# CarbonMatrixLab/AbX

Measured on AMD Instinct MI355X. Metric: diffusion-steps/sec (100 samples, ~350-res complex), higher is better.
Workload: dtype f32; 1 GPU; L352: L=352 (Lab 228 + antigen 124), 100 samples of one complex over 1 GPU(s), 1 step = ScoreNetwork (3 passes) + get_prev + reverse, seeded random weights, ESM off; L=352, samples_total=100, chunk=auto, parallelism=sample-shard x1, no collective in the step

## Files before the change

### abx_amd/csrc/gemm3.hip

```cpp
#include "common.h"
#include "abx_hip.h"
#include "gemm_epilogue.h"
#include "rigid_dev.h"

namespace {

constexpr int BK = 16;
#ifndef ABX_SPLIT_MIN_TILES
#define ABX_SPLIT_MIN_TILES 256
#endif
typedef __attribute__((address_space(3))) void* lds_ptr_t;
typedef const __attribute__((address_space(1))) void* glb_ptr_t;

__device__ __forceinline__ void glds16(const void* src, char* dst_wave_base) {
    __builtin_amdgcn_global_load_lds((glb_ptr_t)src, (lds_ptr_t)dst_wave_base, 16, 0, 0);
}

__device__ __forceinline__ unsigned vgpr32(unsigned o) {
    asm volatile("" : "+v"(o));
    return o;
}

template <int N> __device__ __forceinline__ void wait_vm_and_barrier() {
    asm volatile("s_waitcnt vmcnt(%0) lgkmcnt(0)\n\ts_barrier" ::"n"(N) : "memory");
}

template <int ROWS>
__device__ __forceinline__ int plane_off(int plane, int row, int half) {
    return plane * (ROWS * 32) + row * 32 + ((half ^ ((row >> 3) & 1)) << 4);
}

template <int ROWS, int NL, int NPL = 2>
__device__ __forceinline__ void plane_sources(long long s_plane, long long s_row, int r0, int R, unsigned (&off)[NL]) {
    const int lane = threadIdx.x & 63, wave = threadIdx.x >> 6;
#pragma unroll
    for (int i = 0; i < NL; ++i) {
        int o = (wave * NL + i) * 1024 + lane * 16;
        if (o >= NPL * ROWS * 32) o -= NPL * ROWS * 32;
        const int plane = o / (ROWS * 32), rem = o % (ROWS * 32);
        const int row = rem >> 5, hp = (rem >> 4) & 1;
        const int half = hp ^ ((row >> 3) & 1);
        const int gr = min(r0 + row, R - 1);
        off[i] = (unsigned)((plane * s_plane + (long long)gr * s_row + 8 * half) * 2);
    }
}

template <int BM, int BN, int WM, int WN, int AMODE, bool SWAP = false, bool STATS = true, int RING = 2, int JGO = 0>
__device__ __forceinline__ void gemm3_mainloop(const AbxGemm& g, float* smem, int mt, int nt, int b, f32x16 (&acc)[WM / 32][WN / 32],
                                               float (&ls)[WM / 32], float (&lq)[WM / 32], float (&lshift)[WM / 32],
                                               const char* a_lds = nullptr, int a_lds_stride = 0) {
    constexpr int TM = WM / 32, TN = WN / 32;
    constexpr int WAVES_N = BN / WN;
    constexpr int A_IMG = AMODE == 3 ? 0 : (AMODE == 2 ? 2 * BM * 32 : BM * 64);
    constexpr int NLA = AMODE == 3 ? 1 : (A_IMG + 4095) / 4096;
    constexpr int A_STAGE = RING == 2 ? A_IMG : (A_IMG + 4095) / 4096 * 4096;
    constexpr int B_IMG = 2 * BN * 32;
// ... 528 lines not shown
#pragma unroll
                    for (int q = 0; q < 2; ++q) {
                        const int hc = hid0 + j * 32 + 8 * (2 * s2 + q) + 4 * h;
                        const int hcl = min(hc, MLP_NH - 4);
                        const f32x4 cs = *reinterpret_cast<const f32x4*>(cst + hcl), bi = *reinterpret_cast<const f32x4*>(cst + MLP_NH + hcl);
#pragma unroll
                        for (int e = 0; e < 4; ++e) {
                            float x = rstd * (acc1[0][j][8 * s2 + 4 * q + e] - dmean * cs[e]) + bi[e];
                            x = relu_keep_nan(x);
                            v[4 * q + e] = (hc + e < g.N) ? x : 0.f;
                        }
                    }
                    unsigned q0[4], q1[4];
#pragma unroll
                    for (int e = 0; e < 4; ++e) split2b(v[2 * e], v[2 * e + 1], q0[e], q1[e]);
                    hf[0] = u32x4{q0[0], q0[1], q0[2], q0[3]};
                    hf[1] = u32x4{q1[0], q1[1], q1[2], q1[3]};
                }
                const int kl = 2 * j + s2;
                const int knext = c * (BN / 16) + kl + 1;
                if (kl + 1 < BN / 16 && knext * 16 < g.N) issue_w2(knext, (kl + 1) & 1);
                const char* ws = W2s + (kl & 1) * B2_IMG + offB2;
                if (rows_live && (c * (BN / 16) + kl) * 16 < g.N) {
#pragma unroll
                    for (int t0 = 0; t0 < TN2; t0 += TG2) {
                        u32x4 wb[TG2][2];
#pragma unroll
                        for (int t = 0; t < TG2; ++t)
#pragma unroll
                            for (int p = 0; p < 2; ++p) wb[t][p] = *reinterpret_cast<const u32x4*>(ws + (t0 + t) * 1024 + p * (BN2 * 32));
                        constexpr int TA[3] = {1, 0, 0}, TB[3] = {0, 1, 0};
#pragma unroll
                        for (int term = 0; term < 3; ++term)
#pragma unroll
                            for (int t = 0; t < TG2; ++t)
                                acc2[0][t0 + t] = mfma_split(hf[TA[term]], wb[t][TB[term]], acc2[0][t0 + t]);
                    }
                }
                wait_vm_and_barrier<0>();
            }
        }
    }
    {
        const float cs2 = __builtin_ldexpf(1.0f, -4 - g.b2_exp);
#pragma unroll
        for (int t = 0; t < TN2; ++t) acc2[0][t] *= cs2;
    }
    AbxGemm g2 = g;
    g2.N = g.N2; g2.bias = g.bias2; g2.ln_csum = nullptr; g2.ln_stats = nullptr; g2.act = 0; g2.alpha = 1.0f;
    __syncthreads();
    gemm_epilogue<BM, BN2, WM, BN2, EDGE, false>(g2, smem, smem + 2 * BM, acc2, mt * BM, 0, b, false);
}

template <int MINB>
__global__ __launch_bounds__(256, MINB) void gemm3_mlp_kernel(const AbxGemm g) {
    constexpr int OPER = (2 * 128 * 64 + 2 * 2 * 128 * 32 + 2 * 2 * 192 * 32) / 4 + 2 * MLP_NH;
    constexpr int EPI = 2 * 128 + 4 * 32 * (3 * 32 + 4);
    __shared__ __attribute__((aligned(16))) float smem[OPER > EPI ? OPER : EPI];
    const int ntm = (g.M + 127) / 128;
    const unsigned nwg = gridDim.x, bid = blockIdx.x;
    const unsigned q = nwg >> 3, r = nwg & 7, xcd = bid & 7, loc = bid >> 3;
    const unsigned wgid = (xcd < r ? xcd * (q + 1) : r * (q + 1) + (xcd - r) * q) + loc;
    const int b = (int)(wgid / (unsigned)ntm), mt = (int)(wgid - (unsigned)b * (unsigned)ntm);
    const ClockProbe probe(g.clock_probe);
    if ((mt + 1) * 128 <= g.M && g.N2 == 192) gemm3_mlp_block<false>(g, smem, mt, b);
    else gemm3_mlp_block<true>(g, smem, mt, b);
    probe.finish();
}

constexpr int MLP3_LDS = 3 * (128 * 64 + 2 * 128 * 32) + 2 * 2 * 192 * 32 + 2 * MLP_NH * 4;
__global__ __launch_bounds__(256, 2) void gemm3_mlp3_kernel(const AbxGemm g) {
    extern __shared__ __attribute__((aligned(16))) float mlp3_smem[];
    const int ntm = (g.M + 127) / 128;
    const unsigned nwg = gridDim.x, bid = blockIdx.x;
    const unsigned q = nwg >> 3, r = nwg & 7, xcd = bid & 7, loc = bid >> 3;
    const unsigned wgid = (xcd < r ? xcd * (q + 1) : r * (q + 1) + (xcd - r) * q) + loc;
    const int b = (int)(wgid / (unsigned)ntm), mt = (int)(wgid - (unsigned)b * (unsigned)ntm);
    const ClockProbe probe(g.clock_probe);
    if ((mt + 1) * 128 <= g.M && g.N2 == 192) gemm3_mlp_block<false, 3>(g, mlp3_smem, mt, b);
    else gemm3_mlp_block<true, 3>(g, mlp3_smem, mt, b);
    probe.finish();
}

constexpr int GT_NG = 192;
template <bool EDGE>
__device__ __forceinline__ void gemm3_gtail2w_block(const AbxGemm& g, float* smem, int mt, int b) {
    constexpr int BM = 128, BN = 96, WM = 32, WN = 96, BN2 = 192, TN2 = BN2 / 32;
    constexpr int G1_BYTES = 2 * BM * 64 + 2 * 2 * BN * 32;
    constexpr int B2_IMG = 2 * BN2 * 32;
    constexpr int NL2 = (B2_IMG + 4095) / 4096;
    constexpr int G_IMG = BM * 64;
    char* W2s = reinterpret_cast<char*>(smem) + G1_BYTES;
    char* Gs = W2s + 2 * B2_IMG;
    float* cst = reinterpret_cast<float*>(Gs + 3 * G_IMG);
    for (int i = threadIdx.x; i < GT_NG; i += 256) {
        cst[i] = i < g.N ? g.ln_csum[i] : 0.f;
        cst[GT_NG + i] = (i < g.N && g.bias) ? g.bias[i] : 0.f;
    }
    const int lane = threadIdx.x & 63, wave = __builtin_amdgcn_readfirstlane(threadIdx.x >> 6), h = lane >> 5;
    const int m0 = mt * BM;
    f32x16 acc2[1][TN2];
#pragma unroll
    for (int t = 0; t < TN2; ++t)
#pragma unroll
        for (int r = 0; r < 16; ++r) acc2[0][t][r] = 0.f;
    unsigned offs2[NL2];
    plane_sources<BN2, NL2>(g.sB23p, g.sB23n, 0, g.N2, offs2);
    const char* base2 = reinterpret_cast<const char*>(g.B2_split);
    const long long step2 = g.sB23k * 2;
    unsigned offsG[2];
    const char* baseG = reinterpret_cast<const char*>(g.gate + (long long)b * g.sGb + (long long)m0 * g.sGm);
#pragma unroll
    for (int i = 0; i < 2; ++i) {
        const int r = (wave * 2 + i) * 16 + (lane >> 2), p = lane & 3;
        const int kq = p ^ ((r >> 2) & 3);
        const int gri = min(m0 + r, g.M - 1) - m0;
        offsG[i] = (unsigned)(((long long)gri * g.sGm + kq * 4) * 4);
    }
    static_assert(B2_IMG % 4096 == 0, "uniform DMA instruction counts per wave (counted waits)");
    auto issue_w2 = [&](int ktile) {
        char* dst = W2s + (ktile & 1) * B2_IMG + wave * NL2 * 1024;
        const char* src = base2 + ktile * step2;
#pragma unroll
        for (int i = 0; i < NL2; ++i) glds16(src + vgpr32(offs2[i]), dst + i * 1024);
    };
    const int nkt2 = g.N / 16;
    auto issue_g = [&](int ktile) {
        const int kt = min(ktile, nkt2 - 1);
        char* dg = Gs + (ktile % 3) * G_IMG + wave * 2048;
        const char* sg = baseG + kt * 64;
#pragma unroll
        for (int i = 0; i < 2; ++i) glds16(sg + vgpr32(offsG[i]), dg + i * 1024);
    };
    const int offB2 = plane_off<BN2>(0, lane & 31, h);
// ... 589 lines not shown
    }
    if (!g.A_split && g.sAk == 1 && ((g.a_pair_transpose > 0 || g.a_pair) ? (long long)g.M * g.sAm : 128LL * g.sAm) >= (1LL << 30)) return 1;
    if (g.pair_Lp > 0 && g.c_pair && g.c_transposed) return 1;
    if (g.a_pair && (g.A_split || g.sAk != 1)) return 1;
    if (!g.A_split && g.sAk != 1 && 16LL * g.sAk + g.M >= (1LL << 30)) return 1;
    if (((long long)g.M + 127) / 128 * (((long long)g.N + 127) / 128) * g.batch >= (1LL << 31)) return 1;
    if (g.A_split && (long long)(g.K / 16) * g.sA3k >= (1LL << 31)) return 1;
    if ((long long)(g.K / 16) * g.sB3k >= (1LL << 31)) return 1;
    if (g.out_ln_w) {
        if (g.N > 128 || g.c_transposed || g.C_split || g.A2 || g.A_split || g.sAk != 1 || !g.out_ln_b) {
            abx_set_error("abx_gemm: out_ln needs N <= 128, a k-contiguous fp32 A and a plain store (split-f16 path)");
            *rc = ABX_ERR_ARG;
            return 0;
        }
        const long long mt = ((long long)g.M + 127) / 128;
        hipLaunchKernelGGL((gemm3_oln_kernel<128, 128, 32, 128, 4>), dim3((unsigned)(mt * g.batch)), dim3(256), 0, st, g);
        *rc = abx_check_launch("abx_gemm(out_ln)");
        return 0;
    }
    if (g.mlp == 2) {
        if (g.A_split || g.sAk != 1 || g.c_transposed || g.C_split || g.glu || g.A2 || g.out_ln_w || !g.B2_split || g.N2 <= 0 || g.N2 > 192 ||
            g.N % 16 != 0 || g.N > GT_NG || g.act != 2 || g.alpha != 1.0f || g.rowscale || !g.gate || !g.ln_csum || g.ln_stats || g.a_relu ||
            g.a_pair_transpose > 0 || g.pair_Lp > 0 || !al16(g.B2_split) || g.sB23n % 8 != 0 || g.sB23p % 8 != 0 || g.sB23k % 8 != 0 ||
            (long long)(g.N / 16) * g.sB23k >= (1LL << 31) || !al16(g.ln_csum) || (g.bias && !al16(g.bias)) || !al16(g.gate) || g.sGm % 4 != 0 ||
            g.sGb % 4 != 0 || 128LL * g.sGm >= (1LL << 30)) {
            abx_set_error("abx_gemm: mlp = 2 (gated tail) needs a k-contiguous fp32 A with folded LayerNorm, act = 2, a 16-byte aligned gate "
                          "operand [M][N], N % 16 == 0, N2 <= 192, plain store, B2_split planes in the permuted k order");
            *rc = ABX_ERR_ARG;
            return 0;
        }
        const long long mt = ((long long)g.M + 127) / 128;
        if (g.tune & 64) {
            if (int e = abx_ensure_dynamic_lds(reinterpret_cast<const void*>(&gemm3_gtail2w_kernel), GT_LDS, "abx_gemm(gated tail)")) { *rc = e; return 0; }
            hipLaunchKernelGGL(gemm3_gtail2w_kernel, dim3((unsigned)(mt * g.batch)), dim3(256), GT_LDS, st, g);
            *rc = abx_check_launch("abx_gemm(gated tail, two walks)");
            return 0;
        }
        if (int e = abx_ensure_dynamic_lds(reinterpret_cast<const void*>(&gemm3_gtail_kernel), GT1_LDS, "abx_gemm(gated tail)")) { *rc = e; return 0; }
        hipLaunchKernelGGL(gemm3_gtail_kernel, dim3((unsigned)(mt * g.batch)), dim3(256), GT1_LDS, st, g);
        *rc = abx_check_launch("abx_gemm(gated tail)");
        return 0;
    }
    if (g.mlp) {
        if (g.A_split || g.sAk != 1 || g.c_transposed || g.C_split || g.glu || g.A2 || g.out_ln_w || !g.B2_split || g.N2 <= 0 || g.N2 > 192 ||
            g.N % 16 != 0 || g.N > MLP_NH || g.act != 1 || g.alpha != 1.0f || g.rowscale || g.gate || !g.ln_csum || g.ln_stats || g.a_relu ||
            g.a_pair_transpose > 0 || g.pair_Lp > 0 || !al16(g.B2_split) || g.sB23n % 8 != 0 || g.sB23p % 8 != 0 || g.sB23k % 8 != 0 ||
            (long long)(g.N / 16) * g.sB23k >= (1LL << 31) || !al16(g.ln_csum) || (g.bias && !al16(g.bias))) {
            abx_set_error("abx_gemm: mlp needs a k-contiguous fp32 A with folded LayerNorm, relu, N % 16 == 0, N <= 768, N2 <= 192, plain store, "
                          "B2_split planes in the permuted k order");
            *rc = ABX_ERR_ARG;
            return 0;
        }
        const long long mt = ((long long)g.M + 127) / 128;
        if ((g.tune >> 5) & 1) {
            if (int e = abx_ensure_dynamic_lds(reinterpret_cast<const void*>(&gemm3_mlp3_kernel), MLP3_LDS, "abx_gemm(mlp)")) { *rc = e; return 0; }
            hipLaunchKernelGGL(gemm3_mlp3_kernel, dim3((unsigned)(mt * g.batch)), dim3(256), MLP3_LDS, st, g);
        } else if ((g.tune >> 4) & 1) hipLaunchKernelGGL(gemm3_mlp_kernel<1>, dim3((unsigned)(mt * g.batch)), dim3(256), 0, st, g);
        else hipLaunchKernelGGL(gemm3_mlp_kernel<2>, dim3((unsigned)(mt * g.batch)), dim3(256), 0, st, g);
        *rc = abx_check_launch("abx_gemm(mlp)");
        return 0;
    }
    if (g.A2) {
        if (g.A_split || g.c_transposed || g.glu || !g.B2_split || g.K2 % 16 != 0 || !al16(g.A2) || g.sA2m % 4 != 0 || g.sA2b % 4 != 0 ||
            !al16(g.B2_split) || g.sB23n % 8 != 0 || g.sB23p % 8 != 0 || g.sB23k % 8 != 0 || !g.ln2_csum ||
            (g.pair_Lp > 0 ? (long long)g.pair_L * g.pair_L * g.sA2m : 128LL * g.sA2m) >= (1LL << 30) ||
            (long long)(g.K2 / 16) * g.sB23k >= (1LL << 31)) {
            abx_set_error("abx_gemm: dual (A2 / B2_split) operands do not qualify for the split-f16 dual kernel");
            *rc = ABX_ERR_ARG;
            return 0;
        }
        const long long mt = ((long long)g.M + 127) / 128, ntn = ((long long)g.N + 95) / 96;
        if (g.N > 96 && g.N <= 192 && (g.tune & 128)) hipLaunchKernelGGL(gemm3_dual1_kernel, dim3((unsigned)(mt * g.batch)), dim3(256), 0, st, g);
        else if (g.tune & 1024) hipLaunchKernelGGL((gemm3_dual_kernel<128, 96, 32, 96, 4>), dim3((unsigned)(mt * ntn * g.batch)), dim3(256), 0, st, g);
        else hipLaunchKernelGGL((gemm3_dual_kernel<128, 96, 32, 96, 3>), dim3((unsigned)(mt * ntn * g.batch)), dim3(256), 0, st, g);
        *rc = abx_check_launch("abx_gemm(dual)");
        return 0;
    }
    if (narrow) {
        const long long mt = ((long long)g.M + 127) / 128;
        dim3 grid((unsigned)(mt * g.batch), 1, 1), block(256);
        if ((g.tune >> 9) & 3) {
            const int v = (g.tune >> 9) & 3;
            if (g.c_transposed) { if (v == 1) hipLaunchKernelGGL((gemm3_narrow_ring_kernel<true, 3, 4>), grid, block, 0, st, g); else hipLaunchKernelGGL((gemm3_narrow_ring_kernel<true, 4, 3>), grid, block, 0, st, g); }
            else { if (v == 1) hipLaunchKernelGGL((gemm3_narrow_ring_kernel<false, 3, 4>), grid, block, 0, st, g); else hipLaunchKernelGGL((gemm3_narrow_ring_kernel<false, 4, 3>), grid, block, 0, st, g); }
            *rc = abx_check_launch("abx_gemm(narrow, ring)");
            return 0;
        }
        if (g.c_transposed) hipLaunchKernelGGL((gemm3_kernel<128, 32, 32, 32, 0, true, 6>), grid, block, 0, st, g);
        else hipLaunchKernelGGL((gemm3_kernel<128, 32, 32, 32, 0, false, 6>), grid, block, 0, st, g);
        *rc = abx_check_launch("abx_gemm(narrow)");
        return 0;
    }
    const long long pad128 = ((g.N + 127) / 128) * 128, pad192 = ((g.N + 191) / 192) * 192;
    const int force = (g.tune >> 1) & 7;
    const bool wide = g.glu ? false : force ? force == 2 : (g.A_split ? pad192 <= pad128 : (pad192 <= pad128 && g.N % 128 != 0));
    const long long ntn128 = ((long long)g.N + 127) / 128;
    if (!wide && !g.glu && !force && mt128 * ntn128 * g.batch < 384 && g.M > 64) *rc = launch3<64, 128, 32, 64, 4>(g, st);
    else if (wide) *rc = launch3<128, 192, 32, 192, 3>(g, st);
    else *rc = launch3<128, 128, 32, 128, 4>(g, st);
    return 0;
}

int abx_gemm3_side_dispatch(const AbxGemm& g, const AbxGemm& s2, hipStream_t st, int* rc) {
    auto al16 = [](const void* p) { return (reinterpret_cast<uintptr_t>(p) & 15) == 0; };
    auto plain_a = [&](const AbxGemm& d) {
        return d.B_split && d.b_f16 && !d.A_split && d.A && d.sAk == 1 && d.K % 16 == 0 && al16(d.A) && d.sAm % 4 == 0 && d.sAb % 4 == 0 &&
               al16(d.B_split) && d.sB3n % 8 == 0 && d.sB3p % 8 == 0 && d.sB3k % 8 == 0 && d.sB3b % 8 == 0 && d.b_exp >= -100 && d.b_exp <= 100 &&
               !d.glu && !d.C_split && !d.A2 && !d.out_ln_w && !d.mlp && d.a_pair_transpose <= 0 && d.pair_Lp == 0 && d.batch_inner == 0 &&
               128LL * d.sAm < (1LL << 30) && (long long)(d.K / 16) * d.sB3k < (1LL << 31) && d.exact != 1;
    };
    if (!plain_a(g) || !plain_a(s2)) return 1;
// ... 79 lines not shown
```

### abx_amd/csrc/gemm_as.hip

```cpp
#include <stdlib.h>

#include <type_traits>

#include "common.h"
#include "abx_hip.h"

namespace {

typedef __attribute__((address_space(3))) void* lds_ptr_t;
typedef const __attribute__((address_space(1))) void* glb_ptr_t;

constexpr int AS_BM = 64, AS_BN = 128, AS_NK = 12, AS_RING = 3;
constexpr int AS_KT = 4096;
constexpr int AS_A = AS_NK * AS_KT;
constexpr int AS_STAGE = 2 * AS_BN * 32;
constexpr int AS_HALF = AS_KT / 2;
constexpr int AS_OFF_RING = AS_A;
constexpr int AS_OFF_ST = AS_OFF_RING + AS_RING * AS_STAGE;
constexpr int AS_OFF_CONST = AS_OFF_ST + 4 * 64 * 4;
constexpr int AS_LDS = AS_OFF_CONST + 2 * 1024;

__device__ __forceinline__ void as_glds16(const void* src, char* dst_wave_base) {
    __builtin_amdgcn_global_load_lds((glb_ptr_t)src, (lds_ptr_t)dst_wave_base, 16, 0, 0);
}
__device__ __forceinline__ unsigned as_vgpr32(unsigned o) {
    asm volatile("" : "+v"(o));
    return o;
}
template <int I> using IC = std::integral_constant<int, I>;
template <int I0, int I1, class F> __device__ __forceinline__ void as_static_for(F&& f) {
    if constexpr (I0 < I1) {
        f(IC<I0>{});
        as_static_for<I0 + 1, I1>(f);
    }
}

template <int ROWS> __device__ __forceinline__ int as_plane_off(int plane, int row, int half) {
    return plane * (ROWS * 32) + row * 32 + ((half ^ ((row >> 3) & 1)) << 4);
}

__device__ __forceinline__ long long as_a_row(const AbxGemm& g, int gri) {
    long long gr = gri;
    if (g.a_pair) {
        int pi, pj;
        if (g.c_split_tile) {
            pair_tile_decode(gri, g.pair_Lp, pi, pj);
            pi = min(pi, g.pair_L - 1);
            pj = min(pj, g.pair_L - 1);
        } else {
            pi = gri / g.pair_Lp;
            pj = min(gri - pi * g.pair_Lp, g.pair_L - 1);
        }
        gr = g.a_pair_transpose > 0 ? (long long)pj * g.pair_L + pi : (long long)pi * g.pair_L + pj;
    } else if (g.a_pair_transpose > 0) {
        const int qi = gri / g.a_pair_transpose;
        gr = (long long)(gri - qi * g.a_pair_transpose) * g.a_pair_transpose + qi;
    }
    return gr;
}

__device__ __forceinline__ void as_issue_a(const AbxGemm& g, char* lds, int m0, int b, int wm) {
    const int lane = threadIdx.x & 63;
    const bool remap = g.a_pair_transpose > 0 || g.a_pair != 0;
    const long long row0 = remap ? 0 : m0;
    const char* baseA = reinterpret_cast<const char*>(g.A + (long long)b * g.sAb + row0 * g.sAm);
    unsigned offA[2];
#pragma unroll
    for (int i = 0; i < 2; ++i) {
        const int r = 16 * i + (lane >> 2), p = lane & 3;
        const int kq = p ^ ((r >> 2) & 3);
        const long long gr = as_a_row(g, min(m0 + wm * 32 + r, g.M - 1));
        offA[i] = (unsigned)(((gr - row0) * g.sAm + kq * 4) * 4);
    }
    char* dst = lds + wm * AS_HALF;
#pragma unroll
    for (int kt = 0; kt < AS_NK; ++kt)
#pragma unroll
        for (int i = 0; i < 2; ++i) as_glds16(baseA + kt * 64 + as_vgpr32(offA[i]), dst + kt * AS_KT + i * 1024);
}

struct AsConv {
    float lshift, m2048;
    f32x2 ls2, lq2;
    int rd0, rd1, wr;
    bool ln, relu;
};
__device__ __forceinline__ void as_conv_init(AsConv& c, const AbxGemm& g) {
    const int lane = threadIdx.x & 63, r = lane & 31, h = lane >> 5, x = (r >> 2) & 3;
    c.rd0 = r * 64 + (((2 * h) ^ x) << 4);
    c.rd1 = r * 64 + (((2 * h + 1) ^ x) << 4);
    c.wr = as_plane_off<32>(0, r, h);
    c.lshift = 0.f;
    c.ls2 = c.lq2 = (f32x2){0.f, 0.f};
    c.m2048 = -2048.0f;
    asm volatile("" : "+v"(c.m2048));
    c.ln = g.ln_csum != nullptr;
    c.relu = g.a_relu != 0;
}
template <bool FIRST>
__device__ __forceinline__ void as_conv_ktile(AsConv& c, char* img) {
    const int lane = threadIdx.x & 63;
    const f32x4 lo = *reinterpret_cast<const f32x4*>(img + c.rd0);
    const f32x4 hi = *reinterpret_cast<const f32x4*>(img + c.rd1);
    float xv[8];
#pragma unroll
    for (int e = 0; e < 4; ++e) { xv[e] = lo[e]; xv[4 + e] = hi[e]; }
    if (c.ln) {
        if (FIRST) c.lshift = __shfl(xv[0], lane & 31, 64);
        const f32x2 sh2 = {c.lshift, c.lshift};
#pragma unroll
        for (int e = 0; e < 4; ++e) {
            f32x2 xp = {xv[2 * e], xv[2 * e + 1]};
            xp -= sh2;
            c.ls2 += xp;
            c.lq2 = __builtin_elementwise_fma(xp, xp, c.lq2);
            xv[2 * e] = xp[0];
            xv[2 * e + 1] = xp[1];
        }
    }
    if (c.relu) {
#pragma unroll
        for (int e = 0; e < 8; ++e) xv[e] = fmaxf(xv[e], 0.f);
    }
    unsigned q0[4], q1[4];
#pragma unroll
    for (int e = 0; e < 4; ++e) split2h_mix(xv[2 * e], xv[2 * e + 1], c.m2048, q0[e], q1[e]);
    *reinterpret_cast<u32x4*>(img + c.wr) = u32x4{q0[0], q0[1], q0[2], q0[3]};
    *reinterpret_cast<u32x4*>(img + c.wr + 1024) = u32x4{q1[0], q1[1], q1[2], q1[3]};
}
__device__ __forceinline__ void as_conv_finish(const AsConv& c, float* st, int wm, float eps, float cs) {
    const int lane = threadIdx.x & 63;
    const float ls = c.ls2[0] + c.ls2[1], lq = c.lq2[0] + c.lq2[1];
    const float invK = 1.0f / (float)(AS_NK * 16);
    const float sm = ls + __shfl_xor(ls, 32, 64), sq = lq + __shfl_xor(lq, 32, 64);
    if (lane < 32) {
        const float dm = sm * invK;
        st[wm * 32 + lane] = dm;
        st[64 + wm * 32 + lane] = (1.0f / sqrtf(fmaxf(sq * invK - dm * dm, 0.f) + eps)) * cs;
    }
}

__device__ __forceinline__ void as_quad_transpose(const float (&x)[4], float (&o)[4]) {
    float a0, a1, a2, a3;
    asm volatile(
        "s_nop 1\n\t"
        "s_mov_b32 vcc_lo, 0x55555555\n\ts_mov_b32 vcc_hi, 0x55555555\n\t"
        "v_cndmask_b32_dpp %4, %9, %8, vcc quad_perm:[1,0,3,2] row_mask:0xf bank_mask:0xf\n\t"
        "v_cndmask_b32_dpp %6, %11, %10, vcc quad_perm:[1,0,3,2] row_mask:0xf bank_mask:0xf\n\t"
        "s_mov_b32 vcc_lo, 0xaaaaaaaa\n\ts_mov_b32 vcc_hi, 0xaaaaaaaa\n\t"
        "v_cndmask_b32_dpp %5, %8, %9, vcc quad_perm:[1,0,3,2] row_mask:0xf bank_mask:0xf\n\t"
        "v_cndmask_b32_dpp %7, %10, %11, vcc quad_perm:[1,0,3,2] row_mask:0xf bank_mask:0xf\n\t"
        "s_mov_b32 vcc_lo, 0x33333333\n\ts_mov_b32 vcc_hi, 0x33333333\n\t"
        "v_cndmask_b32_dpp %0, %6, %4, vcc quad_perm:[2,3,0,1] row_mask:0xf bank_mask:0xf\n\t"
        "v_cndmask_b32_dpp %1, %7, %5, vcc quad_perm:[2,3,0,1] row_mask:0xf bank_mask:0xf\n\t"
        "s_mov_b32 vcc_lo, 0xcccccccc\n\ts_mov_b32 vcc_hi, 0xcccccccc\n\t"
        "v_cndmask_b32_dpp %2, %4, %6, vcc quad_perm:[2,3,0,1] row_mask:0xf bank_mask:0xf\n\t"
        "v_cndmask_b32_dpp %3, %5, %7, vcc quad_perm:[2,3,0,1] row_mask:0xf bank_mask:0xf"
        : "=&v"(o[0]), "=&v"(o[1]), "=&v"(o[2]), "=&v"(o[3]), "=&v"(a0), "=&v"(a1), "=&v"(a2), "=&v"(a3)
        : "v"(x[0]), "v"(x[1]), "v"(x[2]), "v"(x[3])
        : "vcc");
}

template <int S0, int NSL, int NST, int NDMA = 4>
struct AsSched {
    static_assert(S0 >= 2 && S0 + NSL <= 10, "slice window");
    static constexpr int after(int kt, bool first) { return (kt == 0 ? 2 : 0) + ((!first && kt >= S0 && kt < S0 + NSL) ? NST : 0); }
    static constexpr int allow(int kt, bool first) {
        const int k2 = (kt + AS_NK - 2) % AS_NK, k1 = (kt + AS_NK - 1) % AS_NK;
        return after(k2, first) + NDMA + after(k1, first);
    }
};

enum { AS_EPI_PLAIN = 0, AS_EPI_GLU = 1 };

template <int N>
__device__ __forceinline__ void as_rendezvous(u32x4 (&fa)[2], u32x4 (&fb)[2][2]) {
    asm volatile("s_waitcnt vmcnt(%6) lgkmcnt(0)\n\ts_barrier"
                 : "+v"(fa[0]), "+v"(fa[1]), "+v"(fb[0][0]), "+v"(fb[0][1]), "+v"(fb[1][0]), "+v"(fb[1][1])
                 : "n"(N)
                 : "memory");
}
__device__ __forceinline__ void as_rendezvous_free(u32x4 (&fa)[2], u32x4 (&fb)[2][2]) {
    asm volatile("s_waitcnt lgkmcnt(0)\n\ts_barrier"
                 : "+v"(fa[0]), "+v"(fa[1]), "+v"(fb[0][0]), "+v"(fb[0][1]), "+v"(fb[1][0]), "+v"(fb[1][1])
                 :
                 : "memory");
}
template <int N> __device__ __forceinline__ void as_wait_vm() { asm volatile("s_waitcnt vmcnt(%0)" ::"n"(N) : "memory"); }

template <int EPI, bool SIDE, bool EDGE, int ABL = 0, bool PL = false>
__device__ __forceinline__ void as_block(const AbxGemm& g, const AbxGemm& s2, char* lds, int mt, int b) {
    const int lane = threadIdx.x & 63, wave = __builtin_amdgcn_readfirstlane(threadIdx.x >> 6);
    const int wm = wave >> 1, wn = wave & 1, h = lane >> 5;
    const int m0 = mt * AS_BM;
    float* st = reinterpret_cast<float*>(lds + AS_OFF_ST);
    using Sched = typename std::conditional<EPI == AS_EPI_PLAIN, AsSched<2, 8, (ABL == 1 ? 0 : (PL ? 2 : 1)), (ABL == 3 ? 2 : 4)>, AsSched<6, 2, (ABL == 1 ? 0 : 2), (ABL == 3 ? 2 : 4)>>::type;

    const int ntiles = (g.N + AS_BN - 1) / AS_BN;
    const bool ragged = (g.N % AS_BN) != 0;
    const char* bbase = reinterpret_cast<const char*>(g.B_split);
    const long long bkstep = g.sB3k * 2;
    unsigned off0, offU[2];
    {
        const int row = lane >> 1, hp = lane & 1;
        off0 = (unsigned)((wm * g.sB3p + (long long)row * g.sB3n + 8 * (hp ^ ((row >> 3) & 1))) * 2);
#pragma unroll
        for (int i = 2; i < 4; ++i) {
            const int r2 = i * 32 + row;
            const int half = hp ^ ((row >> 3) & 1);
            if (SIDE) offU[i - 2] = (unsigned)((wm * s2.sB3p + (long long)min(r2 - 64, s2.N - 1) * s2.sB3n + 8 * half) * 2);
            else offU[i - 2] = (unsigned)((wm * g.sB3p + (long long)min((ntiles - 1) * AS_BN + r2, g.N - 1) * g.sB3n + 8 * half) * 2);
        }
    }
// ... 422 lines not shown
```

Measured before the change: 166.2 sample-steps/s.

## Add persistent 512-thread MLP kernel with streamed weight ring and resident A

```diff
diff --git a/abx_amd/csrc/as_conv.h b/abx_amd/csrc/as_conv.h
--- /dev/null
+++ b/abx_amd/csrc/as_conv.h
@@ -0,0 +1,102 @@
+#pragma once
+#include <type_traits>
+
+#include "common.h"
+#include "abx_hip.h"
+
+namespace {
+
+typedef __attribute__((address_space(3))) void* as_lds_ptr_t;
+typedef const __attribute__((address_space(1))) void* as_glb_ptr_t;
+
+__device__ __forceinline__ void as_glds16(const void* src, char* dst_wave_base) {
+    __builtin_amdgcn_global_load_lds((as_glb_ptr_t)src, (as_lds_ptr_t)dst_wave_base, 16, 0, 0);
+}
+__device__ __forceinline__ unsigned as_vgpr32(unsigned o) {
+    asm volatile("" : "+v"(o));
+    return o;
+}
+template <int I> using IC = std::integral_constant<int, I>;
+template <int I0, int I1, class F> __device__ __forceinline__ void as_static_for(F&& f) {
+    if constexpr (I0 < I1) {
+        f(IC<I0>{});
+        as_static_for<I0 + 1, I1>(f);
+    }
+}
+
+template <int ROWS> __device__ __forceinline__ int as_plane_off(int plane, int row, int half) {
+    return plane * (ROWS * 32) + row * 32 + ((half ^ ((row >> 3) & 1)) << 4);
+}
+
+struct AsConv {
+    float lshift, m2048;
+    f32x2 ls2, lq2;
+    int rd0, rd1, wr;
+    bool ln, relu;
+};
+__device__ __forceinline__ void as_conv_init(AsConv& c, const AbxGemm& g) {
+    const int lane = threadIdx.x & 63, r = lane & 31, h = lane >> 5, x = (r >> 2) & 3;
+    c.rd0 = r * 64 + (((2 * h) ^ x) << 4);
+    c.rd1 = r * 64 + (((2 * h + 1) ^ x) << 4);
+    c.wr = as_plane_off<32>(0, r, h);
+    c.lshift = 0.f;
+    c.ls2 = c.lq2 = (f32x2){0.f, 0.f};
+    c.m2048 = -2048.0f;
+    asm volatile("" : "+v"(c.m2048));
+    c.ln = g.ln_csum != nullptr;
+    c.relu = g.a_relu != 0;
+}
+template <bool FIRST>
+__device__ __forceinline__ void as_conv_ktile(AsConv& c, char* img) {
+    const int lane = threadIdx.x & 63;
+    const f32x4 lo = *reinterpret_cast<const f32x4*>(img + c.rd0);
+    const f32x4 hi = *reinterpret_cast<const f32x4*>(img + c.rd1);
+    float xv[8];
+#pragma unroll
+    for (int e = 0; e < 4; ++e) { xv[e] = lo[e]; xv[4 + e] = hi[e]; }
+    if (c.ln) {
+        if (FIRST) c.lshift = __shfl(xv[0], lane & 31, 64);
+        const f32x2 sh2 = {c.lshift, c.lshift};
+#pragma unroll
+        for (int e = 0; e < 4; ++e) {
+            f32x2 xp = {xv[2 * e], xv[2 * e + 1]};
+            xp -= sh2;
+            c.ls2 += xp;
+            c.lq2 = __builtin_elementwise_fma(xp, xp, c.lq2);
+            xv[2 * e] = xp[0];
+            xv[2 * e + 1] = xp[1];
+        }
+    }
+    if (c.relu) {
+#pragma unroll
+        for (int e = 0; e < 8; ++e) xv[e] = fmaxf(xv[e], 0.f);
+    }
+    unsigned q0[4], q1[4];
+#pragma unroll
+    for (int e = 0; e < 4; ++e) split2h_mix(xv[2 * e], xv[2 * e + 1], c.m2048, q0[e], q1[e]);
+    *reinterpret_cast<u32x4*>(img + c.wr) = u32x4{q0[0], q0[1], q0[2], q0[3]};
+    *reinterpret_cast<u32x4*>(img + c.wr + 1024) = u32x4{q1[0], q1[1], q1[2], q1[3]};
+}
+
+__device__ __forceinline__ void as_quad_transpose(const float (&x)[4], float (&o)[4]) {
+    float a0, a1, a2, a3;
+    asm volatile(
+        "s_nop 1\n\t"
+        "s_mov_b32 vcc_lo, 0x55555555\n\ts_mov_b32 vcc_hi, 0x55555555\n\t"
+        "v_cndmask_b32_dpp %4, %9, %8, vcc quad_perm:[1,0,3,2] row_mask:0xf bank_mask:0xf\n\t"
+        "v_cndmask_b32_dpp %6, %11, %10, vcc quad_perm:[1,0,3,2] row_mask:0xf bank_mask:0xf\n\t"
+        "s_mov_b32 vcc_lo, 0xaaaaaaaa\n\ts_mov_b32 vcc_hi, 0xaaaaaaaa\n\t"
+        "v_cndmask_b32_dpp %5, %8, %9, vcc quad_perm:[1,0,3,2] row_mask:0xf bank_mask:0xf\n\t"
+        "v_cndmask_b32_dpp %7, %10, %11, vcc quad_perm:[1,0,3,2] row_mask:0xf bank_mask:0xf\n\t"
+        "s_mov_b32 vcc_lo, 0x33333333\n\ts_mov_b32 vcc_hi, 0x33333333\n\t"
+        "v_cndmask_b32_dpp %0, %6, %4, vcc quad_perm:[2,3,0,1] row_mask:0xf bank_mask:0xf\n\t"
+        "v_cndmask_b32_dpp %1, %7, %5, vcc quad_perm:[2,3,0,1] row_mask:0xf bank_mask:0xf\n\t"
+        "s_mov_b32 vcc_lo, 0xcccccccc\n\ts_mov_b32 vcc_hi, 0xcccccccc\n\t"
+        "v_cndmask_b32_dpp %2, %4, %6, vcc quad_perm:[2,3,0,1] row_mask:0xf bank_mask:0xf\n\t"
+        "v_cndmask_b32_dpp %3, %5, %7, vcc quad_perm:[2,3,0,1] row_mask:0xf bank_mask:0xf"
+        : "=&v"(o[0]), "=&v"(o[1]), "=&v"(o[2]), "=&v"(o[3]), "=&v"(a0), "=&v"(a1), "=&v"(a2), "=&v"(a3)
+        : "v"(x[0]), "v"(x[1]), "v"(x[2]), "v"(x[3])
+        : "vcc");
+}
+
+}
diff --git a/abx_amd/csrc/gemm3.hip b/abx_amd/csrc/gemm3.hip
--- a/abx_amd/csrc/gemm3.hip
+++ b/abx_amd/csrc/gemm3.hip
@@ -2,6 +2,7 @@
 #include "abx_hip.h"
 #include "gemm_epilogue.h"
 #include "rigid_dev.h"
+#include "mlp_as.h"
 
 namespace {
 
@@ -636,34 +637,27 @@
     gemm_epilogue<BM, BN2, WM, BN2, EDGE, false>(g2, smem, smem + 2 * BM, acc2, mt * BM, 0, b, false);
 }
 
-template <int MINB>
-__global__ __launch_bounds__(256, MINB) void gemm3_mlp_kernel(const AbxGemm g) {
-    constexpr int OPER = (2 * 128 * 64 + 2 * 2 * 128 * 32 + 2 * 2 * 192 * 32) / 4 + 2 * MLP_NH;
-    constexpr int EPI = 2 * 128 + 4 * 32 * (3 * 32 + 4);
-    __shared__ __attribute__((aligned(16))) float smem[OPER > EPI ? OPER : EPI];
-    const int ntm = (g.M + 127) / 128;
-    const unsigned nwg = gridDim.x, bid = blockIdx.x;
-    const unsigned q = nwg >> 3, r = nwg & 7, xcd = bid & 7, loc = bid >> 3;
-    const unsigned wgid = (xcd < r ? xcd * (q + 1) : r * (q + 1) + (xcd - r) * q) + loc;
-    const int b = (int)(wgid / (unsigned)ntm), mt = (int)(wgid - (unsigned)b * (unsigned)ntm);
-    const ClockProbe probe(g.clock_probe);
-    if ((mt + 1) * 128 <= g.M && g.N2 == 192) gemm3_mlp_block<false>(g, smem, mt, b);
-    else gemm3_mlp_block<true>(g, smem, mt, b);
-    probe.finish();
-}
-
-constexpr int MLP3_LDS = 3 * (128 * 64 + 2 * 128 * 32) + 2 * 2 * 192 * 32 + 2 * MLP_NH * 4;
-__global__ __launch_bounds__(256, 2) void gemm3_mlp3_kernel(const AbxGemm g) {
-    extern __shared__ __attribute__((aligned(16))) float mlp3_smem[];
-    const int ntm = (g.M + 127) / 128;
-    const unsigned nwg = gridDim.x, bid = blockIdx.x;
-    const unsigned q = nwg >> 3, r = nwg & 7, xcd = bid & 7, loc = bid >> 3;
-    const unsigned wgid = (xcd < r ? xcd * (q + 1) : r * (q + 1) + (xcd - r) * q) + loc;
-    const int b = (int)(wgid / (unsigned)ntm), mt = (int)(wgid - (unsigned)b * (unsigned)ntm);
-    const ClockProbe probe(g.clock_probe);
-    if ((mt + 1) * 128 <= g.M && g.N2 == 192) gemm3_mlp_block<false, 3>(g, mlp3_smem, mt, b);
-    else gemm3_mlp_block<true, 3>(g, mlp3_smem, mt, b);
-    probe.finish();
+template <int FORM>
+__global__ __launch_bounds__(FORM == 2 ? 512 : 256, FORM == 3 ? 2 : 1) void gemm3_mlp_kernel(const AbxGemm g) {
+    if constexpr (FORM == 2) {
+        extern __shared__ __attribute__((aligned(16))) float mlp_as_smem[];
+        const ClockProbe probe(g.clock_probe);
+        mlp_as_run(g, reinterpret_cast<char*>(mlp_as_smem));
+        probe.finish();
+    } else {
+        constexpr int OPER = (2 * 128 * 64 + 2 * 2 * 128 * 32 + 2 * 2 * 192 * 32) / 4 + 2 * MLP_NH;
+        constexpr int EPI = 2 * 128 + 4 * 32 * (3 * 32 + 4);
+        __shared__ __attribute__((aligned(16))) float smem[OPER > EPI ? OPER : EPI];
+        const int ntm = (g.M + 127) / 128;
+        const unsigned nwg = gridDim.x, bid = blockIdx.x;
+        const unsigned q = nwg >> 3, r = nwg & 7, xcd = bid & 7, loc = bid >> 3;
+        const unsigned wgid = (xcd < r ? xcd * (q + 1) : r * (q + 1) + (xcd - r) * q) + loc;
+        const int b = (int)(wgid / (unsigned)ntm), mt = (int)(wgid - (unsigned)b * (unsigned)ntm);
+        const ClockProbe probe(g.clock_probe);
+        if ((mt + 1) * 128 <= g.M && g.N2 == 192) gemm3_mlp_block<false>(g, smem, mt, b);
+        else gemm3_mlp_block<true>(g, smem, mt, b);
+        probe.finish();
+    }
 }
 
 constexpr int GT_NG = 192;
@@ -1359,11 +1353,24 @@
             return 0;
         }
         const long long mt = ((long long)g.M + 127) / 128;
-        if ((g.tune >> 5) & 1) {
-            if (int e = abx_ensure_dynamic_lds(reinterpret_cast<const void*>(&gemm3_mlp3_kernel), MLP3_LDS, "abx_gemm(mlp)")) { *rc = e; return 0; }
-            hipLaunchKernelGGL(gemm3_mlp3_kernel, dim3((unsigned)(mt * g.batch)), dim3(256), MLP3_LDS, st, g);
-        } else if ((g.tune >> 4) & 1) hipLaunchKernelGGL(gemm3_mlp_kernel<1>, dim3((unsigned)(mt * g.batch)), dim3(256), 0, st, g);
-        else hipLaunchKernelGGL(gemm3_mlp_kernel<2>, dim3((unsigned)(mt * g.batch)), dim3(256), 0, st, g);
+        const bool resident = !(g.tune & (1 << 14)) && g.K == 16 * MA_NK && g.N == MA_NH && g.N2 == MA_N2 && g.c_vec_ok && (!g.resid || g.r_vec_ok) &&
+                              !g.c_pair && !g.a_pair && (!g.bias2 || al16(g.bias2));
+        if ((g.tune >> 4) & 1) hipLaunchKernelGGL(gemm3_mlp_kernel<1>, dim3((unsigned)(mt * g.batch)), dim3(256), 0, st, g);
+        else if (resident) {
+            static int n_cu = 0;
+            if (n_cu == 0) {
+                int dev = 0;
+                hipDeviceProp_t prop;
+                if (hipGetDevice(&dev) != hipSuccess || hipGetDeviceProperties(&prop, dev) != hipSuccess) {
+                    abx_set_error("abx_gemm(mlp): hipGetDeviceProperties failed");
+                    *rc = ABX_ERR_ARG;
+                    return 0;
+                }
+                n_cu = prop.multiProcessorCount > 0 ? prop.multiProcessorCount : 256;
+            }
+            if (int e = abx_ensure_dynamic_lds(reinterpret_cast<const void*>(&gemm3_mlp_kernel<2>), MA_LDS, "abx_gemm(mlp)")) { *rc = e; return 0; }
+            hipLaunchKernelGGL(gemm3_mlp_kernel<2>, dim3((unsigned)n_cu), dim3(512), MA_LDS, st, g);
+        } else hipLaunchKernelGGL(gemm3_mlp_kernel<3>, dim3((unsigned)(mt * g.batch)), dim3(256), 0, st, g);
         *rc = abx_check_launch("abx_gemm(mlp)");
         return 0;
     }
diff --git a/abx_amd/csrc/gemm_as.hip b/abx_amd/csrc/gemm_as.hip
--- a/abx_amd/csrc/gemm_as.hip
+++ b/abx_amd/csrc/gemm_as.hip
@@ -4,6 +4,7 @@
 
 #include "common.h"
 #include "abx_hip.h"
+#include "as_conv.h"
 
 namespace {
 
@@ -19,25 +20,6 @@
 constexpr int AS_OFF_ST = AS_OFF_RING + AS_RING * AS_STAGE;
 constexpr int AS_OFF_CONST = AS_OFF_ST + 4 * 64 * 4;
 constexpr int AS_LDS = AS_OFF_CONST + 2 * 1024;
-
-__device__ __forceinline__ void as_glds16(const void* src, char* dst_wave_base) {
-    __builtin_amdgcn_global_load_lds((glb_ptr_t)src, (lds_ptr_t)dst_wave_base, 16, 0, 0);
-}
-__device__ __forceinline__ unsigned as_vgpr32(unsigned o) {
-    asm volatile("" : "+v"(o));
-    return o;
-}
-template <int I> using IC = std::integral_constant<int, I>;
-template <int I0, int I1, class F> __device__ __forceinline__ void as_static_for(F&& f) {
-    if constexpr (I0 < I1) {
-        f(IC<I0>{});
-        as_static_for<I0 + 1, I1>(f);
-    }
-}
-
-template <int ROWS> __device__ __forceinline__ int as_plane_off(int plane, int row, int half) {
-    return plane * (ROWS * 32) + row * 32 + ((half ^ ((row >> 3) & 1)) << 4);
-}
 
 __device__ __forceinline__ long long as_a_row(const AbxGemm& g, int gri) {
     long long gr = gri;
@@ -79,55 +61,6 @@
         for (int i = 0; i < 2; ++i) as_glds16(baseA + kt * 64 + as_vgpr32(offA[i]), dst + kt * AS_KT + i * 1024);
 }
 
-struct AsConv {
-    float lshift, m2048;
-    f32x2 ls2, lq2;
-    int rd0, rd1, wr;
-    bool ln, relu;
-};
-__device__ __forceinline__ void as_conv_init(AsConv& c, const AbxGemm& g) {
-    const int lane = threadIdx.x & 63, r = lane & 31, h = lane >> 5, x = (r >> 2) & 3;
-    c.rd0 = r * 64 + (((2 * h) ^ x) << 4);
-    c.rd1 = r * 64 + (((2 * h + 1) ^ x) << 4);
-    c.wr = as_plane_off<32>(0, r, h);
-    c.lshift = 0.f;
-    c.ls2 = c.lq2 = (f32x2){0.f, 0.f};
-    c.m2048 = -2048.0f;
-    asm volatile("" : "+v"(c.m2048));
-    c.ln = g.ln_csum != nullptr;
-    c.relu = g.a_relu != 0;
-}
-template <bool FIRST>
-__device__ __forceinline__ void as_conv_ktile(AsConv& c, char* img) {
-    const int lane = threadIdx.x & 63;
-    const f32x4 lo = *reinterpret_cast<const f32x4*>(img + c.rd0);
-    const f32x4 hi = *reinterpret_cast<const f32x4*>(img + c.rd1);
-    float xv[8];
-#pragma unroll
-    for (int e = 0; e < 4; ++e) { xv[e] = lo[e]; xv[4 + e] = hi[e]; }
-    if (c.ln) {
-        if (FIRST) c.lshift = __shfl(xv[0], lane & 31, 64);
-        const f32x2 sh2 = {c.lshift, c.lshift};
-#pragma unroll
-        for (int e = 0; e < 4; ++e) {
-            f32x2 xp = {xv[2 * e], xv[2 * e + 1]};
-            xp -= sh2;
-            c.ls2 += xp;
-            c.lq2 = __builtin_elementwise_fma(xp, xp, c.lq2);
-            xv[2 * e] = xp[0];
-            xv[2 * e + 1] = xp[1];
-        }
-    }
-    if (c.relu) {
-#pragma unroll
-        for (int e = 0; e < 8; ++e) xv[e] = fmaxf(xv[e], 0.f);
-    }
-    unsigned q0[4], q1[4];
-#pragma unroll
-    for (int e = 0; e < 4; ++e) split2h_mix(xv[2 * e], xv[2 * e + 1], c.m2048, q0[e], q1[e]);
-    *reinterpret_cast<u32x4*>(img + c.wr) = u32x4{q0[0], q0[1], q0[2], q0[3]};
-    *reinterpret_cast<u32x4*>(img + c.wr + 1024) = u32x4{q1[0], q1[1], q1[2], q1[3]};
-}
 __device__ __forceinline__ void as_conv_finish(const AsConv& c, float* st, int wm, float eps, float cs) {
     const int lane = threadIdx.x & 63;
     const float ls = c.ls2[0] + c.ls2[1], lq = c.lq2[0] + c.lq2[1];
@@ -138,27 +71,6 @@
         st[wm * 32 + lane] = dm;
         st[64 + wm * 32 + lane] = (1.0f / sqrtf(fmaxf(sq * invK - dm * dm, 0.f) + eps)) * cs;
     }
-}
-
-__device__ __forceinline__ void as_quad_transpose(const float (&x)[4], float (&o)[4]) {
-    float a0, a1, a2, a3;
-    asm volatile(
-        "s_nop 1\n\t"
-        "s_mov_b32 vcc_lo, 0x55555555\n\ts_mov_b32 vcc_hi, 0x55555555\n\t"
-        "v_cndmask_b32_dpp %4, %9, %8, vcc quad_perm:[1,0,3,2] row_mask:0xf bank_mask:0xf\n\t"
-        "v_cndmask_b32_dpp %6, %11, %10, vcc quad_perm:[1,0,3,2] row_mask:0xf bank_mask:0xf\n\t"
-        "s_mov_b32 vcc_lo, 0xaaaaaaaa\n\ts_mov_b32 vcc_hi, 0xaaaaaaaa\n\t"
-        "v_cndmask_b32_dpp %5, %8, %9, vcc quad_perm:[1,0,3,2] row_mask:0xf bank_mask:0xf\n\t"
-        "v_cndmask_b32_dpp %7, %10, %11, vcc quad_perm:[1,0,3,2] row_mask:0xf bank_mask:0xf\n\t"
-        "s_mov_b32 vcc_lo, 0x33333333\n\ts_mov_b32 vcc_hi, 0x33333333\n\t"
-        "v_cndmask_b32_dpp %0, %6, %4, vcc quad_perm:[2,3,0,1] row_mask:0xf bank_mask:0xf\n\t"
-        "v_cndmask_b32_dpp %1, %7, %5, vcc quad_perm:[2,3,0,1] row_mask:0xf bank_mask:0xf\n\t"
-        "s_mov_b32 vcc_lo, 0xcccccccc\n\ts_mov_b32 vcc_hi, 0xcccccccc\n\t"
-        "v_cndmask_b32_dpp %2, %4, %6, vcc quad_perm:[2,3,0,1] row_mask:0xf bank_mask:0xf\n\t"
-        "v_cndmask_b32_dpp %3, %5, %7, vcc quad_perm:[2,3,0,1] row_mask:0xf bank_mask:0xf"
-        : "=&v"(o[0]), "=&v"(o[1]), "=&v"(o[2]), "=&v"(o[3]), "=&v"(a0), "=&v"(a1), "=&v"(a2), "=&v"(a3)
-        : "v"(x[0]), "v"(x[1]), "v"(x[2]), "v"(x[3])
-        : "vcc");
 }
 
 template <int S0, int NSL, int NST, int NDMA = 4>
diff --git a/abx_amd/csrc/mlp_as.h b/abx_amd/csrc/mlp_as.h
--- /dev/null
+++ b/abx_amd/csrc/mlp_as.h
@@ -0,0 +1,297 @@
+#pragma once
+#include "as_conv.h"
+
+namespace {
+
+constexpr int MA_BM = 128, MA_NK = 12, MA_NH = 768, MA_N2 = 192, MA_NCH = 6;
+constexpr int MA_GRP = 2048;
+constexpr int MA_KT = 4 * MA_GRP;
+constexpr int MA_A = MA_NK * MA_KT;
+constexpr int MA_STAGE = 8192, MA_RING = 6, MA_STEPS = 24;
+constexpr int MA_OFF_RING = MA_A;
+constexpr int MA_OFF_X = MA_OFF_RING + 2 * MA_STAGE;
+constexpr int MA_OFF_CST = MA_OFF_RING + MA_RING * MA_STAGE;
+constexpr int MA_OFF_ST = MA_OFF_CST + 2 * MA_NH * 4;
+constexpr int MA_LDS = MA_OFF_ST + 2 * MA_BM * 4;
+constexpr int MA_AHEAD = 6;
+static_assert(MA_STEPS % MA_RING == 0, "the slot of a stage is its step index in the chunk mod the ring");
+static_assert(MA_AHEAD <= MA_RING, "stage s + AHEAD goes to the slot of stage s, whose fragments were read during step s - 1");
+static_assert(MA_LDS <= 160 * 1024, "one block per CU");
+static_assert(8 * 4096 == (MA_RING - 2) * MA_STAGE, "exchange buffers = the four slots the prefetch of the next tile leaves alone");
+
+template <int N>
+__device__ __forceinline__ void ma_rendezvous(bool streamer, u32x4 (&fa)[2], u32x4 (&fb)[2][2]) {
+    if (streamer)
+        asm volatile("s_waitcnt vmcnt(%6) lgkmcnt(0)\n\ts_barrier"
+                     : "+v"(fa[0]), "+v"(fa[1]), "+v"(fb[0][0]), "+v"(fb[0][1]), "+v"(fb[1][0]), "+v"(fb[1][1])
+                     : "n"(N)
+                     : "memory");
+    else
+        asm volatile("s_waitcnt lgkmcnt(0)\n\ts_barrier"
+                     : "+v"(fa[0]), "+v"(fa[1]), "+v"(fb[0][0]), "+v"(fb[0][1]), "+v"(fb[1][0]), "+v"(fb[1][1])
+                     :
+                     : "memory");
+}
+__device__ __forceinline__ void ma_drain_barrier() { asm volatile("s_waitcnt vmcnt(0) lgkmcnt(0)\n\ts_barrier" ::: "memory"); }
+__device__ __forceinline__ void ma_lds_barrier() { asm volatile("s_waitcnt lgkmcnt(0)\n\ts_barrier" ::: "memory"); }
+
+constexpr int ma_allow(int i, bool last) {
+    const int newest = last ? (i + 5 < 25 ? i + 5 : 25) : i + 5;
+    const int n = newest - (i + 1);
+    return 2 * (n < 0 ? 0 : n);
+}
+static_assert(ma_allow(0, false) == 8 && ma_allow(23, false) == 8 && ma_allow(20, true) == 8 && ma_allow(21, true) == 6 && ma_allow(23, true) == 2, "counted waits");
+
+__device__ __forceinline__ void mlp_as_run(const AbxGemm& g, char* lds) {
+    const int lane = threadIdx.x & 63, wave = __builtin_amdgcn_readfirstlane(threadIdx.x >> 6);
+    const int rg = wave & 3, wh = wave >> 2, h = lane >> 5, r32 = lane & 31;
+    const bool streamer = wh != 0;
+    const int ntm = (g.M + MA_BM - 1) / MA_BM;
+    const int total = ntm * g.batch;
+    int tile = (int)blockIdx.x;
+    if (tile >= total) return;
+
+    float* cst = reinterpret_cast<float*>(lds + MA_OFF_CST);
+    float* st = reinterpret_cast<float*>(lds + MA_OFF_ST);
+    for (int i = threadIdx.x; i < MA_NH; i += 512) {
+        cst[i] = g.ln_csum[i];
+        cst[MA_NH + i] = g.bias ? g.bias[i] : 0.f;
+    }
+
+    const int srow = lane >> 1, shalf = (lane & 1) ^ ((srow >> 3) & 1);
+    unsigned offW1[2], offW2;
+#pragma unroll
+    for (int i = 0; i < 2; ++i) offW1[i] = (unsigned)(((rg >> 1) * g.sB3p + (long long)(64 * (rg & 1) + 32 * i + srow) * g.sB3n + 8 * shalf) * 2);
+    offW2 = (unsigned)(((rg & 1) * g.sB23p + (long long)srow * g.sB23n + 8 * shalf) * 2);
+    const char* w1base = reinterpret_cast<const char*>(g.B_split);
+    const char* w2base = reinterpret_cast<const char*>(g.B2_split);
+    const long long w1k = g.sB3k * 2, w1c = 128LL * g.sB3n * 2, w2k = g.sB23k * 2, w2t = 32LL * g.sB23n * 2;
+    auto issue_stage = [&](int c, auto i_) __attribute__((always_inline)) {
+        constexpr int i = decltype(i_)::value;
+        char* dst = lds + MA_OFF_RING + (i % MA_RING) * MA_STAGE + rg * 2048;
+        if constexpr (i < MA_NK) {
+            const char* src = w1base + c * w1c + i * w1k;
+#pragma unroll
+            for (int q = 0; q < 2; ++q) as_glds16(src + as_vgpr32(offW1[q]), dst + q * 1024);
+        } else {
+            constexpr int ks = (i - MA_NK) / 3, cp = (i - MA_NK) % 3;
+            const int swh = rg >> 1;
+            const char* src = w2base + (long long)(c * 8 + swh * 4 + ks) * w2k;
+#pragma unroll
+            for (int q = 0; q < 2; ++q) {
+                const int nt = (2 * cp + q + 3 * swh) % 6;
+                as_glds16(src + nt * w2t + as_vgpr32(offW2), dst + q * 1024);
+            }
+        }
+    };
+
+    unsigned offA[2];
+    const char* baseA = nullptr;
+    auto a_sources = [&](int t) __attribute__((always_inline)) {
+        const int b = t / ntm, m0 = (t - b * ntm) * MA_BM;
+        baseA = reinterpret_cast<const char*>(g.A + (long long)b * g.sAb + (long long)m0 * g.sAm);
+#pragma unroll
+        for (int i = 0; i < 2; ++i) {
+            const int r = 16 * i + (lane >> 2), p = lane & 3;
+            const int kq = p ^ ((r >> 2) & 3);
+            const int gr = min(m0 + rg * 32 + r, g.M - 1) - m0;
+            offA[i] = (unsigned)(((long long)gr * g.sAm + kq * 4) * 4);
+        }
+    };
+    auto issue_a = [&](int kt) __attribute__((always_inline)) {
+        char* dst = lds + kt * MA_KT + rg * MA_GRP;
+#pragma unroll
+        for (int i = 0; i < 2; ++i) as_glds16(baseA + kt * 64 + as_vgpr32(offA[i]), dst + i * 1024);
+    };
+
+    const int offAf = rg * MA_GRP + as_plane_off<32>(0, r32, h);
+    const int offB1 = MA_OFF_RING + as_plane_off<128>(0, wh * 64 + r32, h);
+    const int offB2 = MA_OFF_RING + wh * 4096 + as_plane_off<64>(0, r32, h);
+    u32x4 fa[2][2], fb[2][2][2];
+    auto read_frags = [&](auto i_) __attribute__((always_inline)) {
+        constexpr int i = decltype(i_)::value, set = i & 1, slot = i % MA_RING;
+        if constexpr (i < MA_NK) {
+#pragma unroll
+            for (int p = 0; p < 2; ++p) fa[set][p] = *reinterpret_cast<const u32x4*>(lds + i * MA_KT + offAf + p * 1024);
+#pragma unroll
+            for (int j = 0; j < 2; ++j)
+#pragma unroll
+                for (int p = 0; p < 2; ++p) fb[set][j][p] = *reinterpret_cast<const u32x4*>(lds + offB1 + slot * MA_STAGE + p * 4096 + j * 1024);
+        } else {
+#pragma unroll
+            for (int t = 0; t < 2; ++t)
+#pragma unroll
+                for (int p = 0; p < 2; ++p) fb[set][t][p] = *reinterpret_cast<const u32x4*>(lds + offB2 + slot * MA_STAGE + p * 2048 + t * 1024);
+        }
+    };
+
+    const float cs1 = __builtin_ldexpf(1.0f, -ABX_F16_A_EXP - g.b_exp);
+    const float cs2 = __builtin_ldexpf(1.0f, -4 - g.b2_exp);
+    const float invK = 1.0f / (float)(MA_NK * 16);
+    bool bad = false;
+    AsConv cv;
+
+    if (!streamer) {
+        a_sources(tile);
+#pragma unroll
+        for (int kt = 0; kt < MA_NK; ++kt) issue_a(kt);
+    } else {
+        issue_stage(0, IC<0>{});
+        issue_stage(0, IC<1>{});
+    }
+
+    for (; tile < total; tile += (int)gridDim.x) {
+        const int next = tile + (int)gridDim.x;
+        const bool has_next = next < total;
+        ma_drain_barrier();
+        as_conv_init(cv, g);
+        if (streamer) {
+            issue_stage(0, IC<2>{});
+            issue_stage(0, IC<3>{});
+            issue_stage(0, IC<4>{});
+            issue_stage(0, IC<5>{});
+        } else {
+            as_conv_ktile<true>(cv, lds + rg * MA_GRP);
+            as_conv_ktile<false>(cv, lds + MA_KT + rg * MA_GRP);
+            if (has_next) a_sources(next);
+        }
+        ma_lds_barrier();
+        read_frags(IC<0>{});
+
+        f32x16 acc2[6];
+#pragma unroll
+        for (int a = 0; a < 6; ++a)
+#pragma unroll
+            for (int r = 0; r < 16; ++r) acc2[a][r] = 0.f;
+        float dmean = 0.f, rstd = 0.f;
+
+        auto chunk = [&](int c, auto mode_) __attribute__((always_inline)) {
+            constexpr int MODE = decltype(mode_)::value;
+            f32x16 acc1[2];
+#pragma unroll
+            for (int j = 0; j < 2; ++j)
+#pragma unroll
+                for (int r = 0; r < 16; ++r) acc1[j][r] = 0.f;
+            u32x4 hf[2][2];
+            auto make_h = [&](auto ks_) __attribute__((always_inline)) {
+                constexpr int ks = decltype(ks_)::value, j = ks >> 1, s2 = ks & 1;
+                float v[8];
+#pragma unroll
+                for (int q = 0; q < 2; ++q) {
+                    const int hc = c * 128 + wh * 64 + j * 32 + 8 * (2 * s2 + q) + 4 * h;
+                    const f32x4 cs = *reinterpret_cast<const f32x4*>(cst + hc), bi = *reinterpret_cast<const f32x4*>(cst + MA_NH + hc);
+#pragma unroll
+                    for (int e = 0; e < 4; ++e) v[4 * q + e] = relu_keep_nan(rstd * (acc1[j][8 * s2 + 4 * q + e] - dmean * cs[e]) + bi[e]);
+                }
+                unsigned q0[4], q1[4];
+#pragma unroll
+                for (int e = 0; e < 4; ++e) split2b(v[2 * e], v[2 * e + 1], q0[e], q1[e]);
+                hf[ks & 1][0] = u32x4{q0[0], q0[1], q0[2], q0[3]};
+                hf[ks & 1][1] = u32x4{q1[0], q1[1], q1[2], q1[3]};
+            };
+            as_static_for<0, MA_STEPS>([&](auto i_) __attribute__((always_inline)) {
+                constexpr int i = decltype(i_)::value, set = i & 1;
+                ma_rendezvous<ma_allow(i, MODE == 2)>(streamer, fa[set], fb[set]);
+                if (streamer) {
+                    if constexpr (i + MA_AHEAD < MA_STEPS) issue_stage(c, IC<i + MA_AHEAD>{});
+                    else if constexpr (MODE != 2) issue_stage(c + 1, IC<i + MA_AHEAD - MA_STEPS>{});
+                    else if constexpr (i + MA_AHEAD - MA_STEPS < 2) issue_stage(0, IC<i + MA_AHEAD - MA_STEPS>{});
+                } else if constexpr (MODE == 2 && i < MA_NK) {
+                    if (has_next) issue_a(i);
+                }
+                if constexpr (i + 1 < MA_STEPS) read_frags(IC<i + 1>{});
+                else if constexpr (MODE != 2) read_frags(IC<0>{});
+                if constexpr (MODE == 0 && i + 2 < MA_NK) {
+                    if (!streamer) {
+                        as_conv_ktile<false>(cv, lds + (i + 2) * MA_KT + rg * MA_GRP);
+                        if constexpr (i + 2 == MA_NK - 1) {
+                            const float ls = cv.ls2[0] + cv.ls2[1], lq = cv.lq2[0] + cv.lq2[1];
+                            const float sm = ls + __shfl_xor(ls, 32, 64), sq = lq + __shfl_xor(lq, 32, 64);
+                            if (lane < 32) {
+                                const float dm = sm * invK;
+                                st[rg * 32 + lane] = dm;
+                                st[MA_BM + rg * 32 + lane] = 1.0f / sqrtf(fmaxf(sq * invK - dm * dm, 0.f) + g.ln_eps);
+                            }
+                        }
+                    }
+                }
+                if constexpr (i < MA_NK) {
+                    using T = SplitTerms;
+                    u32x4 bb[2][3];
+#pragma unroll
+                    for (int j = 0; j < 2; ++j) {
+                        bb[j][0] = fb[set][j][0];
+                        bb[j][1] = fb[set][j][1];
+                        bb[j][2] = f16x8_lo(fb[set][j][0]);
+                    }
+#pragma unroll
+                    for (int term = 0; term < T::N; ++term)
+#pragma unroll
+                        for (int j = 0; j < 2; ++j) acc1[j] = mfma_split(bb[j][T::B[term]], fa[set][T::A[term]], acc1[j]);
+                    if constexpr (i == MA_NK - 1) {
+                        if constexpr (MODE == 0) {
+                            dmean = st[rg * 32 + r32];
+                            rstd = st[MA_BM + rg * 32 + r32];
+                        }
+#pragma unroll
+                        for (int j = 0; j < 2; ++j) acc1[j] *= cs1;
+                        make_h(IC<0>{});
+                    }
+                } else {
+                    constexpr int ks = (i - MA_NK) / 3, cp = (i - MA_NK) % 3;
+                    constexpr int TA[3] = {1, 0, 0}, TB[3] = {0, 1, 0};
+#pragma unroll
+                    for (int term = 0; term < 3; ++term)
+#pragma unroll
+                        for (int t = 0; t < 2; ++t) acc2[2 * cp + t] = mfma_split(hf[ks & 1][TA[term]], fb[set][t][TB[term]], acc2[2 * cp + t]);
+                    if constexpr (cp == 1 && ks + 1 < 4) make_h(IC<ks + 1>{});
+                }
+            });
+        };
+        chunk(0, IC<0>{});
+        for (int c = 1; c < MA_NCH - 1; ++c) chunk(c, IC<1>{});
+        chunk(MA_NCH - 1, IC<2>{});
+
+        const int b = tile / ntm, m0 = (tile - b * ntm) * MA_BM;
+        const int mrow = m0 + rg * 32 + 4 * h + (lane & 3);
+        const int ncol = 4 * (r32 >> 2);
+        const float* rd = g.resid ? g.resid + (long long)b * g.sRb + (long long)mrow * g.sRm + ncol : nullptr;
+        float* cw = g.C + (long long)b * g.sCb + (long long)mrow * g.sCm + ncol;
+        f32x4 rv[3][4];
+#pragma unroll
+        for (int r = 0; r < 3; ++r)
+#pragma unroll
+            for (int rq = 0; rq < 4; ++rq) {
+                rv[r][rq] = (f32x4){0.f, 0.f, 0.f, 0.f};
+                if (rd && mrow + 8 * rq < g.M) rv[r][rq] = *reinterpret_cast<const f32x4*>(rd + (long long)(8 * rq) * g.sRm + (3 * wh + r) * 32);
+            }
+        char* xmine = lds + MA_OFF_X + wave * 4096 + lane * 16;
+        const char* xpartner = lds + MA_OFF_X + (wave ^ 4) * 4096 + lane * 16;
+#pragma unroll
+        for (int r = 0; r < 3; ++r) {
+            if (r > 0) ma_lds_barrier();
+#pragma unroll
+            for (int q = 0; q < 4; ++q)
+                *reinterpret_cast<f32x4*>(xmine + q * 1024) = (f32x4){acc2[3 + r][4 * q], acc2[3 + r][4 * q + 1], acc2[3 + r][4 * q + 2], acc2[3 + r][4 * q + 3]};
+            ma_lds_barrier();
+            const int n = (3 * wh + r) * 32 + r32;
+            const float b2 = g.bias2 ? g.bias2[n] : 0.f;
+#pragma unroll
+            for (int rq = 0; rq < 4; ++rq) {
+                const f32x4 pv = *reinterpret_cast<const f32x4*>(xpartner + rq * 1024);
+                float x[4], o[4];
+#pragma unroll
+                for (int e = 0; e < 4; ++e) x[e] = (acc2[r][4 * rq + e] + pv[e]) * cs2 + b2;
+                as_quad_transpose(x, o);
+                f32x4 v = {o[0], o[1], o[2], o[3]};
+                v += rv[r][rq];
+                bad |= __builtin_amdgcn_classf((v[0] + v[1]) + (v[2] + v[3]), 0x207);
+                if (mrow + 8 * rq < g.M) *reinterpret_cast<f32x4*>(cw + (long long)(8 * rq) * g.sCm + (3 * wh + r) * 32) = v;
+            }
+        }
+    }
+    asm volatile("s_waitcnt vmcnt(0)" ::: "memory");
+    if (g.range_flag && __any(bad) && lane == 0) atomicOr(g.range_flag, g.range_tag);
+}
+
+}
```

New measurement: 163.7 sample-steps/s, median of 2. 0.985x the previous value.
